# AlainSchoebi/semantic-bundle-adjustment-colmap

Measured on AMD Instinct MI355X. Metric: residuals+Jacobians/sec and BA-iteration wall-time, 1k cams / 1M pts / 10M obs, higher is better.
Workload: dtype f64

## Files before the change

semantic-bundle-adjustment-colmap_amd/csrc/semantic.hip:

```cpp
#include <hip/hip_runtime.h>

#include <map>

#include <algorithm>
#include <cmath>
#include <cstring>
#include <type_traits>

#include "ba_math.h"
#include "kernels.h"
#include "semantic.h"

namespace miba {

namespace {

constexpr double kMinStep = 1.4901161193847656e-08;

struct SemArgs {
  const SemSample* samples;
  const SemPair* pairs;
  const double* qt;
  const double* cam;
  const uint32_t* img_cam;
// ... 148 lines not shown
  Q[0] = aa + bb - cc - dd; Q[1] = 2.0 * (bc - ad);  Q[2] = 2.0 * (ac + bd);
  Q[3] = 2.0 * (bc + ad);  Q[4] = aa - bb + cc - dd; Q[5] = 2.0 * (cd - ab);
  Q[6] = 2.0 * (bd - ac);  Q[7] = 2.0 * (ab + cd);  Q[8] = aa - bb - cc + dd;
}

[[maybe_unused]] __device__ inline double rcp_refined(double x) {
  double r = __builtin_amdgcn_rcp(x);
  r = fma(r, fma(-x, r, 1.0), r);
  r = fma(r, fma(-x, r, 1.0), r);
  return r;
}

template <int M>
__device__ inline double distortion_gain(const double* K, double r2) {
  constexpr int np = Model<M>::kNumParams;
  double s = 0.0;
  if constexpr (M == kSimpleRadial || M == kRadial) {
#pragma unroll
    for (int k = 3; k < np; ++k) s += fabs(K[k]);
  } else if constexpr (M == kOpenCV) {
#pragma unroll
    for (int k = 4; k < np; ++k) s += fabs(K[k]);
  }
  const double g = 1.0 + r2;
  return 1.0 + s * g * g * g;
}

template <int M>
__device__ inline void world_to_image_fma(const double* K, double u, double v, double* x, double* y) {
#pragma clang fp contract(fast)
  if constexpr (M == kSimplePinhole) {
    *x = K[0] * u + K[1];
    *y = K[0] * v + K[2];
  } else if constexpr (M == kPinhole) {
    *x = K[0] * u + K[2];
    *y = K[1] * v + K[3];
  } else if constexpr (M == kSimpleRadial || M == kRadial) {
    const double r2 = u * u + v * v;
    double rad = K[3] * r2;
    if constexpr (M == kRadial) rad = rad + K[4] * r2 * r2;
    *x = K[0] * (u + u * rad) + K[1];
    *y = K[0] * (v + v * rad) + K[2];
  } else {
    const double k1 = K[4], k2 = K[5], p1 = K[6], p2 = K[7];
    const double u2 = u * u, uv = u * v, v2 = v * v, r2 = u2 + v2;
    const double rad = k1 * r2 + k2 * r2 * r2;
    const double du = u * rad + 2.0 * p1 * uv + p2 * (r2 + 2.0 * u2);
    const double dv = v * rad + 2.0 * p2 * uv + p1 * (r2 + 2.0 * v2);
    *x = K[0] * (u + du) + K[2];
    *y = K[1] * (v + dv) + K[3];
  }
}

__device__ inline void matvec3_t_fma(const double* A, double v0, double v1, double v2, const double* t,
                                     double pp[3]) {
#pragma clang fp contract(fast)
#pragma unroll
  for (int c = 0; c < 3; ++c) pp[c] = A[3 * c] * v0 + A[3 * c + 1] * v1 + A[3 * c + 2] * v2 + t[c];
}

template <int M>
__device__ inline double margin_model_term(const double* K2, const double p[3], double mag) {
  const double iz = 1.0 / p[2];
  const double u = p[0] * iz, v = p[1] * iz;
  return 2e-11 * (fabs(K2[0]) + fabs(K2[1])) * distortion_gain<M>(K2, u * u + v * v) * (1.0 + fabs(u) + fabs(v)) *
         (1.0 + mag * fabs(iz));
}

template <int M, bool FAST = false>
__device__ inline bool resolve(const SemArgs& a, const double p[3], double mag, float label1, const double* K2,
                               const float2* dl2, const PixelCache& pc, double& f, double exk = 0.0) {
  double iz;
  if constexpr (FAST) {
    const double x0 = p[2];
    double r = __builtin_amdgcn_rcp(x0);
    iz = fma(r, fma(-x0, r, 1.0), r);
  } else {
    iz = rcp_refined(p[2]);
  }
  const double u = p[0] * iz, v = p[1] * iz;
  double x, y;
  if constexpr (FAST)
    world_to_image_fma<M>(K2, u, v, &x, &y);
  else
    world_to_image<M>(K2, u, v, &x, &y);
  if (!(fabs(x) < 1e8 && fabs(y) < 1e8 && fabs(u) < 1e6 && fabs(v) < 1e6)) return false;
  double ex;
  if constexpr (FAST) {
    ex = 1e-6 + exk + 1e-11 * (fabs(x) + fabs(y));
  } else {
    const double kscale = (fabs(K2[0]) + fabs(K2[1])) * distortion_gain<M>(K2, u * u + v * v) *
                          (1.0 + fabs(u) + fabs(v)) * (1.0 + mag * fabs(iz));
    ex = 1e-6 + 1e-11 * (kscale + fabs(x) + fabs(y));
  }
  const double fx = floor(x), fy = floor(y);
  const double rx = x - fx, ry = y - fy;
  if (!(fabs(rx - 0.5) > ex && fabs(ry - 0.5) > ex)) return false;
  const int px = (int)fx + (rx > 0.5 ? 1 : 0);
  const int py = (int)fy + (ry > 0.5 ? 1 : 0);
  if (px < 0 || px >= a.W || py < 0 || py >= a.H) {
    f = 0.0;
    return true;
  }
  float2 s;
  if (pc.valid && px == pc.px && py == pc.py) {
    s = make_float2(pc.depth, pc.label);
  } else {
    s = dl2[(size_t)py * a.W + px];
  }
  const double dd = fabs((double)s.x - p[2]) - a.threshold;
  if (!(fabs(dd) > 1e-9 * (1.0 + fabs((double)s.x) + mag))) return false;
  f = (dd > 0.0) ? 0.0 : ((label1 == s.y) ? 0.0 : 1.0);
  return true;
}

struct PairConst {
  double q1[4], t1[3], q2[4], t2[3];
  double uqi[4];
  double ti[3];
  double u2[4];
  double R2[9];
  double C[9];
  double K2[8];
  uint32_t var1, var2, mask1, mask2;
  uint32_t slot, H2, W2, TW2;
  uint64_t roff, toff;
  double pert[28];
  double ood[14];
  double A[16][9];
  double pj[8][3];
  double rho1, rho2, dt1[3], dt2[3];
};

__device__ __forceinline__ SemArgs with_pair(const SemArgs& ak, const PairConst* __restrict__ P) {
  SemArgs a = ak;
  a.H = (int)P->H2;
  a.W = (int)P->W2;
  a.TW = (int)P->TW2;
  return a;
}

__device__ inline void stencil_bounds(const double* q, const double* t, double rel_step, double* rho, double dt[3]) {
  const double nq2 = q[0] * q[0] + q[1] * q[1] + q[2] * q[2] + q[3] * q[3];
  const double nq = sqrt(nq2);
  double r = 0.0;
  for (int k = 0; k < 4; ++k) {
    const double delta = fmax(kMinStep, fabs(q[k]) * rel_step);
    const double d = fmax(fabs((q[k] + delta) - q[k]), fabs(q[k] - (q[k] - delta)));
    const double perp = d * sqrt(fmax(0.0, 1.0 - q[k] * q[k] / nq2));
    const double den = nq - d;
    r = fmax(r, den > 0.0 ? 2.0 * perp / den : INFINITY);
  }
  *rho = r * 1.001;
  for (int k = 0; k < 3; ++k) {
    const double delta = fmax(kMinStep, fabs(t[k]) * rel_step);
    dt[k] = fmax(fabs((t[k] + delta) - t[k]), fabs(t[k] - (t[k] - delta))) * 1.001;
  }
}

__device__ inline void stencil_prep(const double* q1, const double* t1, const double* q2, const double* t2,
                                    double rel_step, int e, PairConst* __restrict__ P) {
  const int m = e >> 1;
  const bool minus = e & 1;
  const int grp = m < 4 ? 0 : (m < 7 ? 1 : (m < 11 ? 2 : 3));
  const int k = m - (grp == 0 ? 0 : (grp == 1 ? 4 : (grp == 2 ? 7 : 11)));
  const double orig = grp == 0 ? q1[k] : (grp == 1 ? t1[k] : (grp == 2 ? q2[k] : t2[k]));
  const double delta = fmax(kMinStep, fabs(orig) * rel_step);
  const double pert = minus ? orig - delta : orig + delta;
  P->pert[e] = pert;
  if (minus) {
    double one_over_delta = 1.0 / delta;
    one_over_delta /= 2;
    P->ood[m] = one_over_delta;
  }
  if (grp == 1 || grp == 3) return;
  const double* q = grp == 0 ? q1 : q2;
  double qq[4] = {q[0], q[1], q[2], q[3]};
  qq[k] = pert;
  double Q[9];
  quat_matrix_un(qq, Q);
  const double in = 1.0 / (qq[0] * qq[0] + qq[1] * qq[1] + qq[2] * qq[2] + qq[3] * qq[3]);
  double* A = P->A[grp == 0 ? e : e - 6];
  if (grp == 0) {
    double u2[4], R2[9];
// ... 24 lines not shown
  const int lane = threadIdx.x & 31;
  if (zero_n && blockIdx.x == 0 && (int)threadIdx.x < nzero) zero_n[threadIdx.x] = 0u;
  if (k >= npairs) return;
  for (int e = lane; e < blk_stride; e += 32) pair_blk[(size_t)k * blk_stride + e] = 0.0;
  if (pair_cnt && lane == 31) pair_cnt[k] = 0u;
  if (lane > 28) return;
  const SemPair pr = pairs[k];
  if (lane < 28) {
    const double* a1 = qt + 8 * (size_t)pr.i;
    const double* a2 = qt + 8 * (size_t)pr.j;
    const double q1[4] = {a1[0], a1[1], a1[2], a1[3]}, t1[3] = {a1[4], a1[5], a1[6]};
    const double q2[4] = {a2[0], a2[1], a2[2], a2[3]}, t2[3] = {a2[4], a2[5], a2[6]};
    stencil_prep(q1, t1, q2, t2, rel_step, lane, out + k);
    return;
  }
  PairConst& P = out[k];
  const double* a1 = qt + 8 * (size_t)pr.i;
  const double* a2 = qt + 8 * (size_t)pr.j;
  for (int m = 0; m < 4; ++m) { P.q1[m] = a1[m]; P.q2[m] = a2[m]; }
  for (int m = 0; m < 3; ++m) { P.t1[m] = a1[4 + m]; P.t2[m] = a2[4 + m]; }
  Pose1Stage s;
  const double zero[3] = {0.0, 0.0, 0.0};
  pose1_stage(P.q1, zero, s);
  {
    const double* q1 = P.q1;
    const double sc = 1.0 / sqrt(q1[0] * q1[0] + q1[1] * q1[1] + q1[2] * q1[2] + q1[3] * q1[3]);
    const double qi[4] = {sc * q1[0], -(sc * q1[1]), -(sc * q1[2]), -(sc * q1[3])};
    const double scale = 1.0 / sqrt(qi[0] * qi[0] + qi[1] * qi[1] + qi[2] * qi[2] + qi[3] * qi[3]);
    for (int m = 0; m < 4; ++m) P.uqi[m] = scale * qi[m];
  }
  P.ti[0] = -(s.R[0] * P.t1[0] + s.R[1] * P.t1[1] + s.R[2] * P.t1[2]);
  P.ti[1] = -(s.R[3] * P.t1[0] + s.R[4] * P.t1[1] + s.R[5] * P.t1[2]);
  P.ti[2] = -(s.R[6] * P.t1[0] + s.R[7] * P.t1[1] + s.R[8] * P.t1[2]);
  unit_quat(P.q2, P.u2);
  unit_quat_matrix(P.u2, P.R2);
  for (int r = 0; r < 3; ++r)
    for (int c = 0; c < 3; ++c)
      P.C[3 * r + c] = P.R2[3 * r] * s.R[c] + P.R2[3 * r + 1] * s.R[3 + c] + P.R2[3 * r + 2] * s.R[6 + c];
  const double* K = cam + 8 * (size_t)img_cam[pr.j];
  for (int m = 0; m < 8; ++m) P.K2[m] = K[m];
  P.var1 = pr.var1;
  P.var2 = pr.var2;
  P.mask1 = (img_flags[pr.i] >> 1) & 7u;
  P.mask2 = (img_flags[pr.j] >> 1) & 7u;
  P.slot = raster_slot[pr.j];
  const SlotInfo si = slots[P.slot];
  P.H2 = (uint32_t)si.H;
  P.W2 = (uint32_t)si.W;
  P.TW2 = (uint32_t)si.TW;
  P.roff = si.off;
  P.toff = si.toff;
  stencil_bounds(P.q1, P.t1, rel_step, &P.rho1, P.dt1);
  stencil_bounds(P.q2, P.t2, rel_step, &P.rho2, P.dt2);
}

constexpr int kPairVals = 78 + 12;
constexpr int kPairStride = 96;
constexpr int kSemRow = 13;

template <int M>
__device__ __forceinline__ double stencil_reference(const SemArgs& a, const PairConst* __restrict__ P, int grp, int k,
                                                 double pert, const double pc1[3], float label1, const double* K2,
                                                 const float2* dl2) {
  double qq1[4], tt1[3], qq2[4], tt2[3];
#pragma unroll
  for (int c = 0; c < 4; ++c) {
    qq1[c] = (grp == 0 && c == k) ? pert : P->q1[c];
    qq2[c] = (grp == 2 && c == k) ? pert : P->q2[c];
  }
#pragma unroll
  for (int c = 0; c < 3; ++c) {
    tt1[c] = (grp == 1 && c == k) ? pert : P->t1[c];
    tt2[c] = (grp == 3 && c == k) ? pert : P->t2[c];
  }
  int st2;
  return semantic_error<M>(a, pc1, label1, qq1, tt1, qq2, tt2, K2, dl2, &st2);
}

template <bool FAST, int GRP>
__device__ __forceinline__ void stencil_pp(const PairConst* __restrict__ P, int e, int k, const double w[3],
                                           const double pw[3], const double p2[3], double pp[3]) {
  if constexpr (GRP == 0 || GRP == 2) {
    const double* A = P->A[GRP == 0 ? e : e - 6];
    const double* v = GRP == 0 ? w : pw;
    if constexpr (FAST) {
      matvec3_t_fma(A, v[0], v[1], v[2], P->t2, pp);
    } else {
#pragma unroll
      for (int c = 0; c < 3; ++c) pp[c] = A[3 * c] * v[0] + A[3 * c + 1] * v[1] + A[3 * c + 2] * v[2] + P->t2[c];
    }
  } else if constexpr (GRP == 1) {
    const double dt = P->pert[e] - P->t1[k];
#pragma unroll
    for (int c = 0; c < 3; ++c) pp[c] = p2[c] - dt * P->C[3 * c + k];
  } else {
    const double dt = P->pert[e] - P->t2[k];
#pragma unroll
    for (int c = 0; c < 3; ++c) pp[c] = p2[c] + (c == k ? dt : 0.0);
  }
}

template <int M, bool FAST, int GRP>
__device__ __forceinline__ double stencil_point(const SemArgs& a, const PairConst* __restrict__ P, int e, int k,
                                                const double w[3], const double pw[3], const double p2[3],
                                                double mag, const double pc1[3], float label1, const double* K2,
                                                const float2* dl2, const PixelCache& pc, double exk) {
// ... 370 lines not shown
  for (int k = 0; k < nc; ++k) gm = fmax(gm, fmax(cu[k], cv[k]));
  if (!(gm < 0.1)) return false;
  const double ru = fabs(u) + gm, rv = fabs(v) + gm;
  const double H = second_derivative_bound<M>(K2, sqrt(ru * ru + rv * rv) * (1.0 + 1e-12));
  const double fx = fabs(K2[0]);
  const double fy = (M == kPinhole || M == kOpenCV) ? fabs(K2[1]) : fabs(K2[0]);
  double bxm = 0.0, bym = 0.0;
  for (int k = 0; k < nc; ++k) {
    const double sk = cu[k] + cv[k];
    bxm = fmax(bxm, (fabs(A[0]) + fx * H * sk) * cu[k] + (fabs(A[1]) + fx * H * sk) * cv[k]);
    bym = fmax(bym, (fabs(A[2]) + fy * H * sk) * cu[k] + (fabs(A[3]) + fy * H * sk) * cv[k]);
  }
  const double gain = distortion_gain<M>(K2, u * u + v * v);
  const double kscale = (fabs(K2[0]) + fabs(K2[1])) * gain * (1.0 + fabs(u) + fabs(v)) * (1.0 + c.mag * fabs(iz));
  const double ex = 1e-6 + 1e-11 * (kscale + fabs(x) + fabs(y));
  const double bx = bxm * (1.0 + 1e-12) + ex;
  const double by = bym * (1.0 + 1e-12) + ex;
  fb.x0 = (int)round(x - bx);
  fb.y0 = (int)round(y - by);
  fb.ncol = (int)round(x + bx) - fb.x0 + 1;
  fb.nrow = (int)round(y + by) - fb.y0 + 1;
  fb.d = az_max;
  return fb.ncol <= 3 && fb.nrow <= 3;
}

template <int M>
__device__ __forceinline__ void image_jac_bound(const double* K, double u, double v, double Ah[4]) {
  const double r2 = u * u + v * v, r1 = fabs(u) + fabs(v);
  if constexpr (M == kSimplePinhole) {
    Ah[0] = Ah[3] = fabs(K[0]);
    Ah[1] = Ah[2] = 0.0;
  } else if constexpr (M == kPinhole) {
    Ah[0] = fabs(K[0]);
    Ah[3] = fabs(K[1]);
    Ah[1] = Ah[2] = 0.0;
  } else if constexpr (M == kSimpleRadial) {
    const double k = fabs(K[3]);
    Ah[0] = Ah[3] = fabs(K[0]) * (1.0 + 3.0 * k * r2);
    Ah[1] = Ah[2] = fabs(K[0]) * (k * r2);
  } else if constexpr (M == kRadial) {
    const double k1 = fabs(K[3]), k2 = fabs(K[4]);
    Ah[0] = Ah[3] = fabs(K[0]) * (1.0 + 3.0 * k1 * r2 + 5.0 * k2 * r2 * r2);
    Ah[1] = Ah[2] = fabs(K[0]) * (k1 * r2 + 2.0 * k2 * r2 * r2);
  } else {
    const double k1 = fabs(K[4]), k2 = fabs(K[5]), p1 = fabs(K[6]), p2 = fabs(K[7]);
    const double rad = 3.0 * k1 * r2 + 5.0 * k2 * r2 * r2, off = k1 * r2 + 2.0 * k2 * r2 * r2 + 2.0 * (p1 + p2) * r1;
    Ah[0] = fabs(K[0]) * (1.0 + rad + (2.0 * p1 + 6.0 * p2) * r1);
    Ah[1] = fabs(K[0]) * off;
    Ah[2] = fabs(K[1]) * off;
    Ah[3] = fabs(K[1]) * (1.0 + rad + (6.0 * p1 + 2.0 * p2) * r1);
  }
}

template <int M, bool EXACT_A = false, bool GROUPS = false>
__device__ __forceinline__ bool flat_box_coarse(const PairConst* __restrict__ P, const Centre& c, const double* K2,
                                                double u, double v, double x, double y, FlatBox& fb) {
  const double z = c.p2[2];
  if (!(z > 0.0)) return false;
  double Ae[4];
  if constexpr (EXACT_A) {
    constexpr int np = Model<M>::kNumParams;
    double Jp[2 * np];
    world_to_image_jac<M>(K2, u, v, &x, &y, Ae, Jp);
  }
  if (!(fabs(x) < 1e8 && fabs(y) < 1e8 && fabs(u) < 1e6 && fabs(v) < 1e6)) return false;
  double dq = 0.0, tx = 0.0, ty = 0.0, tz = 0.0;
  if (P->var1) {
    dq = P->rho1 * sqrt(c.w[0] * c.w[0] + c.w[1] * c.w[1] + c.w[2] * c.w[2]) * (1.0 + 1e-12);
    tx = fmax(P->dt1[0] * fabs(P->C[0]), fmax(P->dt1[1] * fabs(P->C[1]), P->dt1[2] * fabs(P->C[2])));
    ty = fmax(P->dt1[0] * fabs(P->C[3]), fmax(P->dt1[1] * fabs(P->C[4]), P->dt1[2] * fabs(P->C[5])));
    tz = fmax(P->dt1[0] * fabs(P->C[6]), fmax(P->dt1[1] * fabs(P->C[7]), P->dt1[2] * fabs(P->C[8])));
  }
  if (P->var2) {
    dq = fmax(dq, P->rho2 * sqrt(c.pw[0] * c.pw[0] + c.pw[1] * c.pw[1] + c.pw[2] * c.pw[2]) * (1.0 + 1e-12));
    tx = fmax(tx, P->dt2[0]);
    ty = fmax(ty, P->dt2[1]);
    tz = fmax(tz, P->dt2[2]);
  }
  const double az = fmax(dq, tz);
  if (!(z - az > 0.5 * z)) return false;
  const double iden = 1.0 / (z - az) * (1.0 + 1e-12);
  const double cu_r = (dq + fabs(u) * dq) * iden, cv_r = (dq + fabs(v) * dq) * iden;
  const double cu_t = (tx + fabs(u) * tz) * iden, cv_t = (ty + fabs(v) * tz) * iden;
  const double cu = fmax(cu_r, cu_t), cv = fmax(cv_r, cv_t);
  const double gm = fmax(cu, cv);
  if (!(gm < 0.1)) return false;
  const double ru = fabs(u) + gm, rv = fabs(v) + gm;
  const double H = second_derivative_bound<M>(K2, sqrt(ru * ru + rv * rv) * (1.0 + 1e-12));
  const double fx = fabs(K2[0]);
  const double fy = (M == kPinhole || M == kOpenCV) ? fabs(K2[1]) : fabs(K2[0]);
  double Ah[4];
  if constexpr (EXACT_A) {
#pragma unroll
    for (int k = 0; k < 4; ++k) Ah[k] = fabs(Ae[k]);
  } else {
    image_jac_bound<M>(K2, u, v, Ah);
  }
  double bxm, bym;
  if constexpr (GROUPS) {
    const double sr = cu_r + cv_r, st = cu_t + cv_t;
    bxm = fmax((Ah[0] + fx * H * sr) * cu_r + (Ah[1] + fx * H * sr) * cv_r,
               (Ah[0] + fx * H * st) * cu_t + (Ah[1] + fx * H * st) * cv_t);
    bym = fmax((Ah[2] + fy * H * sr) * cu_r + (Ah[3] + fy * H * sr) * cv_r,
               (Ah[2] + fy * H * st) * cu_t + (Ah[3] + fy * H * st) * cv_t);
  } else {
    const double sk = cu + cv;
    bxm = (Ah[0] + fx * H * sk) * cu + (Ah[1] + fx * H * sk) * cv;
    bym = (Ah[2] + fy * H * sk) * cu + (Ah[3] + fy * H * sk) * cv;
  }
  const double gain = distortion_gain<M>(K2, u * u + v * v);
  const double kscale = (fabs(K2[0]) + fabs(K2[1])) * gain * (1.0 + fabs(u) + fabs(v)) * (1.0 + c.mag * fabs(1.0 / z));
  const double ex = 1e-6 + 1e-11 * (kscale + fabs(x) + fabs(y));
  const double bx = bxm * (1.0 + 1e-12) + ex;
  const double by = bym * (1.0 + 1e-12) + ex;
  fb.x0 = (int)round(x - bx);
  fb.y0 = (int)round(y - by);
  fb.ncol = (int)round(x + bx) - fb.x0 + 1;
  fb.nrow = (int)round(y + by) - fb.y0 + 1;
  fb.d = az;
  return fb.ncol <= 3 && fb.nrow <= 3;
}

__device__ __forceinline__ int flat_index(const SemArgs& a, const FlatBox& fb, bool cand, int q) {
  const int px = fb.x0 + q % 3, py = fb.y0 + q / 3;
  const bool in = cand && q % 3 < fb.ncol && q / 3 < fb.nrow && px >= 0 && px < a.W && py >= 0 && py < a.H;
  return in ? py * a.W + px : 0;
}

__device__ __forceinline__ bool flat_check(const SemArgs& a, const FlatBox& fb, const float2 s[9], double z,
                                           double mag, float label1, double r) {
  bool flat = true;
#pragma unroll
  for (int q = 0; q < 9; ++q) {
    const int px = fb.x0 + q % 3, py = fb.y0 + q / 3;
    if (q % 3 < fb.ncol && q / 3 < fb.nrow) {
      double f = 0.0;
      if (px >= 0 && px < a.W && py >= 0 && py < a.H) {
        const double dz = fabs((double)s[q].x - z) - a.threshold;
        if (!(fabs(dz) > fb.d + 1e-9 * (1.0 + fabs((double)s[q].x) + mag))) flat = false;
        f = dz > 0.0 ? 0.0 : (label1 == s[q].y ? 0.0 : 1.0);
      }
      if (f != r) flat = false;
    }
  }
  return flat;
}

template <int M>
__device__ __forceinline__ bool stencil_flat(const SemArgs& a, const PairConst* __restrict__ P, const Centre& c,
                                             float label1, const double* K2, const float2* __restrict__ dl2) {
  FlatBox fb;
  if (!flat_box<M>(P, c, K2, fb)) return false;
  float2 s[9];
#pragma unroll
  for (int q = 0; q < 9; ++q) s[q] = dl2[flat_index(a, fb, true, q)];
  return flat_check(a, fb, s, c.p2[2], c.mag, label1, c.r);
}

template <int M, bool FAST = false, int NB = 0, bool FLAT = false>
__global__ __launch_bounds__(kBlock) void semantic_linearize_kernel(SemArgs ak, const SemTile* __restrict__ tiles,
                                                                     const PairConst* __restrict__ pcs,
                                                                     double* __restrict__ pair_blk,
                                                                     double* __restrict__ cost_partial,
                                                                     double* __restrict__ r_out,
                                                                     int32_t* __restrict__ status_out,
                                                                     double* __restrict__ J_out, int write_samples) {
  constexpr int kHalf = kBlock / 2;
  constexpr int kBuf = FLAT ? kBlock * 12 : kHalf * kSemRow;
  __shared__ double sbuf[kBuf];
  __shared__ double spart[2 * kPairVals];
  __shared__ double sred[4];
// ... 181 lines not shown
    if (cur == 0ull) {
      const unsigned long long prev = atomicCAS(keys + h, 0ull, key);
      if (prev == 0ull || prev == key) return;
    }
  }
  atomicOr(overflow, 1u);
}

__global__ __launch_bounds__(256) void label_index_kernel(const float2* __restrict__ dl, int64_t n,
                                                          const unsigned long long* __restrict__ keys,
                                                          uint8_t* __restrict__ lab8) {
  const int64_t k = (int64_t)blockIdx.x * 256 + threadIdx.x;
  if (k >= n) return;
  const uint32_t bits = __float_as_uint(dl[k].y);
  const unsigned long long key = (unsigned long long)bits | (1ull << 32);
  uint32_t h = pal_hash(bits);
  for (int probe = 0; probe < 256 && keys[h] != key; ++probe) h = (h + 1u) & 255u;
  lab8[k] = (uint8_t)h;
}

__global__ __launch_bounds__(256) void depth_tile_kernel(const float2* __restrict__ dl,
                                                         const SlotInfo* __restrict__ slots, float2* __restrict__ out) {
  const SlotInfo si = slots[blockIdx.y];
  const int H = si.H, W = si.W, TW = si.TW, TH = (H + 7) / 8;
  const int rem = (int)(blockIdx.x * 256 + threadIdx.x);
  if (rem >= TH * TW) return;
  const int64_t k = (int64_t)si.toff + rem;
  const int ty = rem / TW, tx = rem - ty * TW;
  const float2* base = dl + si.off;
  float dmin = __builtin_inff(), dmax = -__builtin_inff();
  bool nan = false;
  const int y1 = min(8 * ty + 10, H), x1 = min(8 * tx + 10, W);
  for (int y = 8 * ty; y < y1; ++y)
    for (int x = 8 * tx; x < x1; ++x) {
      const float d = base[(int64_t)y * W + x].x;
      nan = nan || d != d;
      dmin = fminf(dmin, d);
      dmax = fmaxf(dmax, d);
    }
  out[k] = nan ? make_float2(__builtin_nanf(""), __builtin_nanf("")) : make_float2(dmin, dmax);
}

__device__ __forceinline__ int tile_depth_side(const SemArgs& a, const FlatBox& fb, float2 dr, double z, double mag) {
  const double dmin = (double)dr.x, dmax = (double)dr.y;
  if (!(dmin <= dmax)) return 0;
  const double margin = fb.d + 1e-9 * (1.0 + fmax(fabs(dmin), fabs(dmax)) + mag);
  const double far = fmax(fabs(dmax - z), fabs(dmin - z));
  if (a.threshold - far > margin) return 1;
  const double nearest = (z >= dmin && z <= dmax) ? 0.0 : fmin(fabs(dmin - z), fabs(dmax - z));
  if (nearest - a.threshold > margin) return 2;
  return 0;
}

template <int M, bool FAST, bool WS = false, bool LP = false, int COARSE = 0>
__global__ __launch_bounds__(kBlock) void semantic_flat_kernel(SemArgs ak, const SemTile* __restrict__ tiles,
                                                               const PairConst* __restrict__ pcs,
                                                               unsigned long long* __restrict__ dmask,
                                                               double* __restrict__ cost_partial,
                                                               double* __restrict__ r_out,
                                                               int32_t* __restrict__ status_out,
                                                               double* __restrict__ J_out, int write_samples) {
  __shared__ double sred[kBlock / 64];
  __shared__ float spal[LP ? 256 : 1];
  const SemTile t = tiles[blockIdx.x];
  const PairConst* __restrict__ P = pcs + t.pair;
  const SemArgs a = with_pair(ak, P);
  const int tid = threadIdx.x, lane = tid & 63;
  const bool active = tid < (int)t.count;
  const int64_t n = (int64_t)t.start + tid;
  const float2* dl2 = a.dl + P->roff;
  const double* K2 = P->K2;
  double cost = 0.0;
  bool deferred = false;
  if constexpr (LP) {
    static_assert(kBlock >= 256, "one palette entry per thread");
    spal[tid] = a.pal[tid];
    __syncthreads();
  }
  if (active) {
    const SemSample smp = a.samples[n];
    Centre c;
    double rot[3];
    unit_quat_rotate(P->uqi, smp.pc1, rot);
    c.pw[0] = rot[0] + P->ti[0];
    c.pw[1] = rot[1] + P->ti[1];
    c.pw[2] = rot[2] + P->ti[2];
    double rot2[3];
    unit_quat_rotate(P->u2, c.pw, rot2);
    c.p2[0] = rot2[0] + P->t2[0];
    c.p2[1] = rot2[1] + P->t2[1];
    c.p2[2] = rot2[2] + P->t2[2];
    c.mag = fabs(smp.pc1[0]) + fabs(smp.pc1[1]) + fabs(smp.pc1[2]) + fabs(P->t1[0]) + fabs(P->t1[1]) +
            fabs(P->t1[2]) + fabs(c.pw[0]) + fabs(c.pw[1]) + fabs(c.pw[2]) + fabs(P->t2[0]) + fabs(P->t2[1]) +
            fabs(P->t2[2]);
    c.w[0] = smp.pc1[0] - P->t1[0];
    c.w[1] = smp.pc1[1] - P->t1[1];
    c.w[2] = smp.pc1[2] - P->t1[2];
    const double u2 = c.p2[0] / c.p2[2];
    const double v2 = c.p2[1] / c.p2[2];
    double x2, y2;
    world_to_image<M>(K2, u2, v2, &x2, &y2);
    const int cpx = cast_to_int_x86(round(x2));
    const int cpy = cast_to_int_x86(round(y2));
    const bool cin = !(cpx < 0 || cpx >= a.W || cpy < 0 || cpy >= a.H);
    FlatBox fb;
    const bool cand = COARSE == 3   ? flat_box_coarse<M, false, true>(P, c, K2, u2, v2, x2, y2, fb)
                      : COARSE == 2 ? flat_box_coarse<M, true>(P, c, K2, u2, v2, x2, y2, fb)
                      : COARSE == 1 ? flat_box_coarse<M>(P, c, K2, u2, v2, x2, y2, fb)
                                    : flat_box<M>(P, c, K2, fb);
    bool decided = false;
    bool resolved = false;
    if constexpr (LP) {
      if (cand && fb.x0 >= 0 && fb.y0 >= 0 && fb.x0 + fb.ncol <= a.W && fb.y0 + fb.nrow <= a.H && cpx >= fb.x0 &&
          cpx < fb.x0 + fb.ncol && cpy >= fb.y0 && cpy < fb.y0 + fb.nrow) {
        const float2 dr = a.dtile[P->toff + (size_t)(fb.y0 >> 3) * a.TW + (fb.x0 >> 3)];
        const uint8_t* lp = a.lab8 + P->roff + (size_t)fb.y0 * a.W + fb.x0;
        const uint8_t lc = lp[(size_t)(cpy - fb.y0) * a.W + (cpx - fb.x0)];
        uint8_t L[9];
#pragma unroll
        for (int q = 0; q < 9; ++q) L[q] = (q % 3 < fb.ncol && q / 3 < fb.nrow) ? lp[(size_t)(q / 3) * a.W + q % 3] : lc;
        const int side = tile_depth_side(a, fb, dr, c.p2[2], c.mag);
        if (side == 2) {
          c.st = MI_BA_INVALID_DEPTH;
          c.r = 0.0;
          decided = resolved = true;
        } else if (side == 1) {
          c.st = MI_BA_VALID;
          c.r = (smp.label1 == spal[lc]) ? 0.0 : 1.0;
          bool flat = true;
#pragma unroll
          for (int q = 0; q < 9; ++q) flat = flat && ((smp.label1 == spal[L[q]]) ? 0.0 : 1.0) == c.r;
          resolved = true;
          decided = flat;
          deferred = !flat;
        }
      }
    }
    if constexpr (WS) {
      if (!resolved && cand && fb.x0 >= 0 && fb.y0 >= 0 && fb.x0 + 2 < a.W && fb.y0 + 2 < a.H) {
        const float4 w = a.wsum[P->roff + (size_t)fb.y0 * a.W + fb.x0];
        decided = resolved = window_decides(a, fb, w, c.p2[2], c.mag, smp.label1, &c.st, &c.r);
      }
    }
    if (!resolved && cand &&
        (fb.x0 + fb.ncol <= 0 || fb.x0 >= a.W || fb.y0 + fb.nrow <= 0 || fb.y0 >= a.H)) {
      c.st = MI_BA_OUT_OF_BOUNDS;
      c.r = 0.0;
      decided = resolved = true;
    }
    if (!resolved) {
      const float2 sc = dl2[cin ? cpy * a.W + cpx : 0];
      float2 s[9];
#pragma unroll
      for (int q = 0; q < 9; ++q) s[q] = dl2[flat_index(a, fb, cand, q)];
      if (!cin) {
        c.st = MI_BA_OUT_OF_BOUNDS;
        c.r = 0.0;
      } else if (fabs((double)sc.x - c.p2[2]) > a.threshold) {
        c.st = MI_BA_INVALID_DEPTH;
        c.r = 0.0;
      } else {
        c.st = MI_BA_VALID;
        c.r = (smp.label1 == sc.y) ? 0.0 : 1.0;
      }
      deferred = !(cand && flat_check(a, fb, s, c.p2[2], c.mag, smp.label1, c.r));
    }
    double rho[3];
    loss_eval(a.loss_type, a.loss_scale, c.r * c.r, rho);
    cost = 0.5 * (a.weight * rho[0]);
    if (write_samples) {
      r_out[n] = c.r;
      status_out[n] = c.st + ((write_samples & 2) && deferred ? 0x1000 : 0) + ((write_samples & 4) && decided ? 0x4000 : 0);
      if (!deferred) {
        double2* jo = reinterpret_cast<double2*>(J_out + 12 * n);
#pragma unroll
        for (int m = 0; m < 6; ++m) jo[m] = make_double2(0.0, 0.0);
      }
    }
  }
  const unsigned long long bal = __ballot(deferred);
  if (lane == 0) dmask[(size_t)blockIdx.x * (kBlock / 64) + (tid >> 6)] = bal;
  double v = cost;
  for (int off = 32; off > 0; off >>= 1) v += __shfl_xor(v, off, 64);
  if (lane == 0) sred[tid >> 6] = v;
  __syncthreads();
  if (tid == 0) {
    double s = 0.0;
#pragma unroll
    for (int w = 0; w < kBlock / 64; ++w) s += sred[w];
    cost_partial[blockIdx.x] = s;
  }
}

template <int M, bool FAST, int NB, bool BOX = false, int WPE = 1>
__global__ __launch_bounds__(64, WPE) void semantic_deferred_kernel(SemArgs ak, const uint2* __restrict__ chunks,
                                                              const uint32_t* __restrict__ ccount,
                                                              const PairConst* __restrict__ pcs,
                                                              const uint32_t* __restrict__ pair_cnt,
                                                              const uint32_t* __restrict__ dlist,
                                                              const uint32_t* __restrict__ pair_chunk0,
                                                              double* __restrict__ cpart,
                                                              double* __restrict__ J_out, int write_samples,
                                                              int32_t* __restrict__ status_out = nullptr) {
  __shared__ double sJ[64 * kSemRow];
  __shared__ float2 sbox[BOX ? 64 * 9 : 1];
  const uint32_t nch = ccount ? *ccount : blockIdx.x + 1;
  const uint32_t stride = ccount ? gridDim.x : 1u;
  for (uint32_t ci = blockIdx.x; ci < nch; ci += stride) {
  const uint2 ch = chunks[ci];
  const uint32_t cnt = pair_cnt[ch.x];
  if (ch.y >= cnt) continue;
  const PairConst* __restrict__ P = pcs + ch.x;
  const SemArgs a = with_pair(ak, P);
  const int lane = threadIdx.x;
  const uint32_t k = ch.y + lane;
  const uint32_t pstart = a.pairs[ch.x].start;
  const float2* dl2 = a.dl + P->roff;
  const double* K2 = P->K2;
  double rowv[kSemRow];
#pragma unroll
  for (int q = 0; q < kSemRow; ++q) rowv[q] = 0.0;
  if (k < cnt) {
    const int64_t n = (int64_t)pstart + dlist[pstart + k];
    const SemSample smp = a.samples[n];
    Centre c;
// ... 1015 lines not shown
```

Measured before the change: 18.93 billion.

## Streamline flat-pixel classifier with precomputed pair bounds and fast approximate math

The per-sample centre projection now uses the precomputed composite rotation C as a single matvec, plus hardware reciprocal with one Newton step and a float sqrt upper bound, instead of two quaternion rotations and exact division. Per-pair stencil bounds and camera-magnitude terms are hoisted into PairConst. The bound routine is merged into one templated function with widened safety margins. Samples near rounding or threshold boundaries fall back to the exact reference path, which trades fewer FLOPs per sample for extra branches and more code.

```diff
diff --git a/semantic-bundle-adjustment-colmap_amd/csrc/semantic.hip b/semantic-bundle-adjustment-colmap_amd/csrc/semantic.hip
--- a/semantic-bundle-adjustment-colmap_amd/csrc/semantic.hip
+++ b/semantic-bundle-adjustment-colmap_amd/csrc/semantic.hip
@@ -224,6 +224,61 @@
   }
 }
 
+template <int M>
+__device__ __forceinline__ void image_point_jac_fma(const double* K, double u, double v, double* x, double* y,
+                                                    double A[4], double* r2o) {
+#pragma clang fp contract(fast)
+  const double u2 = u * u, v2 = v * v, r2 = u2 + v2;
+  *r2o = r2;
+  if constexpr (M == kSimplePinhole) {
+    *x = K[0] * u + K[1];
+    *y = K[0] * v + K[2];
+    A[0] = A[3] = K[0];
+    A[1] = A[2] = 0.0;
+  } else if constexpr (M == kPinhole) {
+    *x = K[0] * u + K[2];
+    *y = K[1] * v + K[3];
+    A[0] = K[0];
+    A[3] = K[1];
+    A[1] = A[2] = 0.0;
+  } else if constexpr (M == kSimpleRadial || M == kRadial) {
+    const double f = K[0];
+    double rad = K[3] * r2, g = 2.0 * K[3];
+    if constexpr (M == kRadial) {
+      rad = rad + K[4] * r2 * r2;
+      g = g + 4.0 * K[4] * r2;
+    }
+    *x = f * (u + u * rad) + K[1];
+    *y = f * (v + v * rad) + K[2];
+    const double guv = g * u * v;
+    A[0] = f * (1.0 + rad + g * u2);
+    A[1] = A[2] = f * guv;
+    A[3] = f * (1.0 + rad + g * v2);
+  } else {
+    const double k1 = K[4], k2 = K[5], p1 = K[6], p2 = K[7];
+    const double uv = u * v;
+    const double rad = r2 * (k1 + k2 * r2);
+    const double g = 2.0 * k1 + 4.0 * k2 * r2;
+    const double tp = 2.0 * (p1 * u + p2 * v);
+    *x = K[0] * (u + u * rad + 2.0 * p1 * uv + p2 * (r2 + 2.0 * u2)) + K[2];
+    *y = K[1] * (v + v * rad + 2.0 * p2 * uv + p1 * (r2 + 2.0 * v2)) + K[3];
+    const double off = g * uv + tp;
+    A[0] = K[0] * (1.0 + rad + g * u2 + 2.0 * p1 * v + 6.0 * p2 * u);
+    A[1] = K[0] * off;
+    A[2] = K[1] * off;
+    A[3] = K[1] * (1.0 + rad + g * v2 + 2.0 * p2 * u + 6.0 * p1 * v);
+  }
+}
+
+__device__ __forceinline__ double rcp_newton1(double x) {
+  const double r = __builtin_amdgcn_rcp(x);
+  return fma(r, fma(-x, r, 1.0), r);
+}
+
+__device__ __forceinline__ double sqrt_upper(double s) {
+  return fma((double)__builtin_amdgcn_sqrtf((float)s), 1.0 + 1e-6, 1e-18);
+}
+
 __device__ inline void matvec3_t_fma(const double* A, double v0, double v1, double v2, const double* t,
                                      double pp[3]) {
 #pragma clang fp contract(fast)
@@ -302,6 +357,11 @@
   double A[16][9];
   double pj[8][3];
   double rho1, rho2, dt1[3], dt2[3];
+  double frho, ftx, fty, ftz;
+  double fk01;
+  double fks[3];
+  double fh6[2], fh20[2], fh3;
+  double ft12;
 };
 
 __device__ __forceinline__ SemArgs with_pair(const SemArgs& ak, const PairConst* __restrict__ P) {
@@ -432,6 +492,33 @@
   P.toff = si.toff;
   stencil_bounds(P.q1, P.t1, rel_step, &P.rho1, P.dt1);
   stencil_bounds(P.q2, P.t2, rel_step, &P.rho2, P.dt2);
+  double rho = 0.0, tx = 0.0, ty = 0.0, tz = 0.0;
+  if (pr.var1) {
+    rho = P.rho1;
+    tx = fmax(P.dt1[0] * fabs(P.C[0]), fmax(P.dt1[1] * fabs(P.C[1]), P.dt1[2] * fabs(P.C[2])));
+    ty = fmax(P.dt1[0] * fabs(P.C[3]), fmax(P.dt1[1] * fabs(P.C[4]), P.dt1[2] * fabs(P.C[5])));
+    tz = fmax(P.dt1[0] * fabs(P.C[6]), fmax(P.dt1[1] * fabs(P.C[7]), P.dt1[2] * fabs(P.C[8])));
+  }
+  if (pr.var2) {
+    rho = fmax(rho, P.rho2);
+    tx = fmax(tx, P.dt2[0]);
+    ty = fmax(ty, P.dt2[1]);
+    tz = fmax(tz, P.dt2[2]);
+  }
+  P.frho = rho;
+  P.ftx = tx;
+  P.fty = ty;
+  P.ftz = tz;
+  P.fk01 = fabs(K[0]) + fabs(K[1]);
+  P.fks[0] = fabs(K[3]);
+  P.fks[1] = fabs(K[3]) + fabs(K[4]);
+  P.fks[2] = fabs(K[4]) + fabs(K[5]) + fabs(K[6]) + fabs(K[7]);
+  P.fh6[0] = 6.0 * fabs(K[3]);
+  P.fh6[1] = 6.0 * fabs(K[4]);
+  P.fh20[0] = 20.0 * fabs(K[4]);
+  P.fh20[1] = 20.0 * fabs(K[5]);
+  P.fh3 = 6.0 * (fabs(K[6]) + fabs(K[7]));
+  P.ft12 = fabs(P.t1[0]) + fabs(P.t1[1]) + fabs(P.t1[2]) + fabs(P.t2[0]) + fabs(P.t2[1]) + fabs(P.t2[2]);
 }
 
 constexpr int kPairVals = 78 + 12;
@@ -908,71 +995,101 @@
   }
 }
 
-template <int M, bool EXACT_A = false, bool GROUPS = false>
-__device__ __forceinline__ bool flat_box_coarse(const PairConst* __restrict__ P, const Centre& c, const double* K2,
-                                                double u, double v, double x, double y, FlatBox& fb) {
-  const double z = c.p2[2];
+struct FlatCentre {
+  double z, u, v, x, y, A[4];
+  double nw;
+  double mag;
+  double m1;
+  double ex;
+};
+
+template <int M, int COARSE>
+__device__ __forceinline__ bool flat_bound(const PairConst* __restrict__ P, const double* K2, const FlatCentre& c,
+                                           FlatBox& fb) {
+#pragma clang fp contract(fast)
+  const double z = c.z;
   if (!(z > 0.0)) return false;
-  double Ae[4];
-  if constexpr (EXACT_A) {
-    constexpr int np = Model<M>::kNumParams;
-    double Jp[2 * np];
-    world_to_image_jac<M>(K2, u, v, &x, &y, Ae, Jp);
-  }
-  if (!(fabs(x) < 1e8 && fabs(y) < 1e8 && fabs(u) < 1e6 && fabs(v) < 1e6)) return false;
-  double dq = 0.0, tx = 0.0, ty = 0.0, tz = 0.0;
-  if (P->var1) {
-    dq = P->rho1 * sqrt(c.w[0] * c.w[0] + c.w[1] * c.w[1] + c.w[2] * c.w[2]) * (1.0 + 1e-12);
-    tx = fmax(P->dt1[0] * fabs(P->C[0]), fmax(P->dt1[1] * fabs(P->C[1]), P->dt1[2] * fabs(P->C[2])));
-    ty = fmax(P->dt1[0] * fabs(P->C[3]), fmax(P->dt1[1] * fabs(P->C[4]), P->dt1[2] * fabs(P->C[5])));
-    tz = fmax(P->dt1[0] * fabs(P->C[6]), fmax(P->dt1[1] * fabs(P->C[7]), P->dt1[2] * fabs(P->C[8])));
-  }
-  if (P->var2) {
-    dq = fmax(dq, P->rho2 * sqrt(c.pw[0] * c.pw[0] + c.pw[1] * c.pw[1] + c.pw[2] * c.pw[2]) * (1.0 + 1e-12));
-    tx = fmax(tx, P->dt2[0]);
-    ty = fmax(ty, P->dt2[1]);
-    tz = fmax(tz, P->dt2[2]);
-  }
-  const double az = fmax(dq, tz);
-  if (!(z - az > 0.5 * z)) return false;
-  const double iden = 1.0 / (z - az) * (1.0 + 1e-12);
-  const double cu_r = (dq + fabs(u) * dq) * iden, cv_r = (dq + fabs(v) * dq) * iden;
-  const double cu_t = (tx + fabs(u) * tz) * iden, cv_t = (ty + fabs(v) * tz) * iden;
-  const double cu = fmax(cu_r, cu_t), cv = fmax(cv_r, cv_t);
-  const double gm = fmax(cu, cv);
-  if (!(gm < 0.1)) return false;
-  const double ru = fabs(u) + gm, rv = fabs(v) + gm;
-  const double H = second_derivative_bound<M>(K2, sqrt(ru * ru + rv * rv) * (1.0 + 1e-12));
+  if (!(fabs(c.x) < 1e8 && fabs(c.y) < 1e8 && fabs(c.u) < 1e6 && fabs(c.v) < 1e6 && c.m1 < 1e3)) return false;
+  const double dq = P->frho * c.nw;
+  const double az = fmax(dq, P->ftz);
+  const double zl = (z - az) - 1e-11 * c.mag;
+  if (!(zl > 0.5 * z)) return false;
+  const double iden = rcp_newton1(zl) * (1.0 + 1e-9);
+  const double eu = 1e-8 * fabs(c.u) + 1e-8, ev = 1e-8 * fabs(c.v) + 1e-8;
+  const double ua = fabs(c.u) + eu, va = fabs(c.v) + ev;
   const double fx = fabs(K2[0]);
   const double fy = (M == kPinhole || M == kOpenCV) ? fabs(K2[1]) : fabs(K2[0]);
+  auto second = [&](double gm) {
+    const double ru = ua + gm, rv = va + gm;
+    const double rho = sqrt_upper(ru * ru + rv * rv);
+    if constexpr (M == kSimpleRadial) return P->fh6[0] * rho;
+    else if constexpr (M == kRadial) return P->fh6[0] * rho + P->fh20[0] * rho * rho * rho;
+    else if constexpr (M == kOpenCV) return P->fh6[1] * rho + P->fh20[1] * rho * rho * rho + P->fh3;
+    else return 0.0;
+  };
   double Ah[4];
-  if constexpr (EXACT_A) {
-#pragma unroll
-    for (int k = 0; k < 4; ++k) Ah[k] = fabs(Ae[k]);
+  if constexpr (COARSE == 1 || COARSE == 3) {
+    image_jac_bound<M>(K2, ua, va, Ah);
   } else {
-    image_jac_bound<M>(K2, u, v, Ah);
+#pragma unroll
+    for (int k = 0; k < 4; ++k) Ah[k] = fabs(c.A[k]);
   }
   double bxm, bym;
-  if constexpr (GROUPS) {
-    const double sr = cu_r + cv_r, st = cu_t + cv_t;
-    bxm = fmax((Ah[0] + fx * H * sr) * cu_r + (Ah[1] + fx * H * sr) * cv_r,
-               (Ah[0] + fx * H * st) * cu_t + (Ah[1] + fx * H * st) * cv_t);
-    bym = fmax((Ah[2] + fy * H * sr) * cu_r + (Ah[3] + fy * H * sr) * cv_r,
-               (Ah[2] + fy * H * st) * cu_t + (Ah[3] + fy * H * st) * cv_t);
+  if constexpr (COARSE == 0) {
+    double cu[7], cv[7];
+    int nc = 0;
+    auto cls = [&](double ax, double ay, double azk) {
+      cu[nc] = (ax + ua * azk) * iden + eu;
+      cv[nc] = (ay + va * azk) * iden + ev;
+      ++nc;
+    };
+    cls(dq, dq, dq);
+    if (P->var1) {
+#pragma unroll
+      for (int k = 0; k < 3; ++k)
+        cls(P->dt1[k] * fabs(P->C[k]), P->dt1[k] * fabs(P->C[3 + k]), P->dt1[k] * fabs(P->C[6 + k]));
+    }
+    if (P->var2) {
+      cls(P->dt2[0], 0.0, 0.0);
+      cls(0.0, P->dt2[1], 0.0);
+      cls(0.0, 0.0, P->dt2[2]);
+    }
+    double gm = 0.0;
+    for (int k = 0; k < nc; ++k) gm = fmax(gm, fmax(cu[k], cv[k]));
+    if (!(gm < 0.1)) return false;
+    const double H = second(gm);
+    bxm = bym = 0.0;
+    for (int k = 0; k < nc; ++k) {
+      const double sk = cu[k] + cv[k];
+      bxm = fmax(bxm, (Ah[0] + fx * H * sk) * cu[k] + (Ah[1] + fx * H * sk) * cv[k]);
+      bym = fmax(bym, (Ah[2] + fy * H * sk) * cu[k] + (Ah[3] + fy * H * sk) * cv[k]);
+    }
   } else {
-    const double sk = cu + cv;
-    bxm = (Ah[0] + fx * H * sk) * cu + (Ah[1] + fx * H * sk) * cv;
-    bym = (Ah[2] + fy * H * sk) * cu + (Ah[3] + fy * H * sk) * cv;
-  }
-  const double gain = distortion_gain<M>(K2, u * u + v * v);
-  const double kscale = (fabs(K2[0]) + fabs(K2[1])) * gain * (1.0 + fabs(u) + fabs(v)) * (1.0 + c.mag * fabs(1.0 / z));
-  const double ex = 1e-6 + 1e-11 * (kscale + fabs(x) + fabs(y));
-  const double bx = bxm * (1.0 + 1e-12) + ex;
-  const double by = bym * (1.0 + 1e-12) + ex;
-  fb.x0 = (int)round(x - bx);
-  fb.y0 = (int)round(y - by);
-  fb.ncol = (int)round(x + bx) - fb.x0 + 1;
-  fb.nrow = (int)round(y + by) - fb.y0 + 1;
+    const double cu_r = (dq + ua * dq) * iden + eu, cv_r = (dq + va * dq) * iden + ev;
+    const double cu_t = (P->ftx + ua * P->ftz) * iden + eu, cv_t = (P->fty + va * P->ftz) * iden + ev;
+    const double cu = fmax(cu_r, cu_t), cv = fmax(cv_r, cv_t);
+    const double gm = fmax(cu, cv);
+    if (!(gm < 0.1)) return false;
+    const double H = second(gm);
+    const double hx = fx * H, hy = fy * H;
+    if constexpr (COARSE == 3) {
+      const double sr = cu_r + cv_r, st = cu_t + cv_t;
+      bxm = fmax((Ah[0] + hx * sr) * cu_r + (Ah[1] + hx * sr) * cv_r,
+                 (Ah[0] + hx * st) * cu_t + (Ah[1] + hx * st) * cv_t);
+      bym = fmax((Ah[2] + hy * sr) * cu_r + (Ah[3] + hy * sr) * cv_r,
+                 (Ah[2] + hy * st) * cu_t + (Ah[3] + hy * st) * cv_t);
+    } else {
+      const double sk = cu + cv;
+      bxm = (Ah[0] + hx * sk) * cu + (Ah[1] + hx * sk) * cv;
+      bym = (Ah[2] + hy * sk) * cu + (Ah[3] + hy * sk) * cv;
+    }
+  }
+  const double bx = bxm * (1.0 + 1e-9) + 2.0 * c.ex;
+  const double by = bym * (1.0 + 1e-9) + 2.0 * c.ex;
+  fb.x0 = (int)floor((c.x - bx) + 0.5);
+  fb.y0 = (int)floor((c.y - by) + 0.5);
+  fb.ncol = (int)floor((c.x + bx) + 0.5) - fb.x0 + 1;
+  fb.nrow = (int)floor((c.y + by) + 0.5) - fb.y0 + 1;
   fb.d = az;
   return fb.ncol <= 3 && fb.nrow <= 3;
 }
@@ -1260,6 +1377,18 @@
   return 0;
 }
 
+__device__ __forceinline__ void reference_point(const PairConst* __restrict__ P, const double pc1[3], double p2[3]) {
+  double rot[3], pw[3], rot2[3];
+  unit_quat_rotate(P->uqi, pc1, rot);
+  pw[0] = rot[0] + P->ti[0];
+  pw[1] = rot[1] + P->ti[1];
+  pw[2] = rot[2] + P->ti[2];
+  unit_quat_rotate(P->u2, pw, rot2);
+  p2[0] = rot2[0] + P->t2[0];
+  p2[1] = rot2[1] + P->t2[1];
+  p2[2] = rot2[2] + P->t2[2];
+}
+
 template <int M, bool FAST, bool WS = false, bool LP = false, int COARSE = 0>
 __global__ __launch_bounds__(kBlock) void semantic_flat_kernel(SemArgs ak, const SemTile* __restrict__ tiles,
                                                                const PairConst* __restrict__ pcs,
@@ -1287,35 +1416,56 @@
   }
   if (active) {
     const SemSample smp = a.samples[n];
-    Centre c;
-    double rot[3];
-    unit_quat_rotate(P->uqi, smp.pc1, rot);
-    c.pw[0] = rot[0] + P->ti[0];
-    c.pw[1] = rot[1] + P->ti[1];
-    c.pw[2] = rot[2] + P->ti[2];
-    double rot2[3];
-    unit_quat_rotate(P->u2, c.pw, rot2);
-    c.p2[0] = rot2[0] + P->t2[0];
-    c.p2[1] = rot2[1] + P->t2[1];
-    c.p2[2] = rot2[2] + P->t2[2];
-    c.mag = fabs(smp.pc1[0]) + fabs(smp.pc1[1]) + fabs(smp.pc1[2]) + fabs(P->t1[0]) + fabs(P->t1[1]) +
-            fabs(P->t1[2]) + fabs(c.pw[0]) + fabs(c.pw[1]) + fabs(c.pw[2]) + fabs(P->t2[0]) + fabs(P->t2[1]) +
-            fabs(P->t2[2]);
-    c.w[0] = smp.pc1[0] - P->t1[0];
-    c.w[1] = smp.pc1[1] - P->t1[1];
-    c.w[2] = smp.pc1[2] - P->t1[2];
-    const double u2 = c.p2[0] / c.p2[2];
-    const double v2 = c.p2[1] / c.p2[2];
-    double x2, y2;
-    world_to_image<M>(K2, u2, v2, &x2, &y2);
-    const int cpx = cast_to_int_x86(round(x2));
-    const int cpy = cast_to_int_x86(round(y2));
+    const double w0 = smp.pc1[0] - P->t1[0], w1 = smp.pc1[1] - P->t1[1], w2 = smp.pc1[2] - P->t1[2];
+    FlatCentre fc;
+    fc.nw = sqrt_upper(fma(w2, w2, fma(w1, w1, w0 * w0)));
+    fc.mag = fma(1.7321, fc.nw, fabs(smp.pc1[0]) + fabs(smp.pc1[1]) + fabs(smp.pc1[2]) + P->ft12);
+    int st = 0;
+    double r = 0.0;
+    double p2[3];
+    matvec3_t_fma(P->C, w0, w1, w2, P->t2, p2);
+    double iz = rcp_newton1(p2[2]);
+    fc.u = p2[0] * iz;
+    fc.v = p2[1] * iz;
+    double r2;
+    image_point_jac_fma<M>(K2, fc.u, fc.v, &fc.x, &fc.y, fc.A, &r2);
+    int cpx, cpy;
+    bool slow;
+    {
+      fc.m1 = fma(fc.mag, fabs(iz), 1.0);
+      const double g1 = 1.0 + r2;
+      const double ks = (M == kSimpleRadial ? P->fks[0] : M == kRadial ? P->fks[1] : M == kOpenCV ? P->fks[2] : 0.0);
+      const double gain = fma(ks, g1 * g1 * g1, 1.0);
+      const double kscale = P->fk01 * gain * (1.0 + fabs(fc.u) + fabs(fc.v)) * fc.m1;
+      fc.ex = 1e-6 + fma(2e-11, kscale, 1e-11 * (fabs(fc.x) + fabs(fc.y)));
+      const double fx = floor(fc.x), fy = floor(fc.y);
+      const double rx = fc.x - fx, ry = fc.y - fy;
+      slow = !(fabs(fc.x) < 1e8 && fabs(fc.y) < 1e8 && fabs(fc.u) < 1e6 && fabs(fc.v) < 1e6 &&
+               fabs(rx - 0.5) > fc.ex && fabs(ry - 0.5) > fc.ex);
+      cpx = (int)fx + (rx > 0.5 ? 1 : 0);
+      cpy = (int)fy + (ry > 0.5 ? 1 : 0);
+    }
+    if (slow) {
+      reference_point(P, smp.pc1, p2);
+      fc.u = p2[0] / p2[2];
+      fc.v = p2[1] / p2[2];
+      double xf, yf;
+      image_point_jac_fma<M>(K2, fc.u, fc.v, &xf, &yf, fc.A, &r2);
+      world_to_image<M>(K2, fc.u, fc.v, &fc.x, &fc.y);
+      cpx = cast_to_int_x86(round(fc.x));
+      cpy = cast_to_int_x86(round(fc.y));
+      if (!(fc.ex < 1e300)) {
+        fc.m1 = fma(fc.mag, fabs(1.0 / p2[2]), 1.0);
+        fc.ex = 1e-6 + 2e-11 * P->fk01 * distortion_gain<M>(K2, fc.u * fc.u + fc.v * fc.v) *
+                           (1.0 + fabs(fc.u) + fabs(fc.v)) * fc.m1 + 1e-11 * (fabs(fc.x) + fabs(fc.y));
+      }
+    }
+    fc.z = p2[2];
+    bool exact_z = false;
+    float cdepth = 0.f, clabel = 0.f;
     const bool cin = !(cpx < 0 || cpx >= a.W || cpy < 0 || cpy >= a.H);
     FlatBox fb;
-    const bool cand = COARSE == 3   ? flat_box_coarse<M, false, true>(P, c, K2, u2, v2, x2, y2, fb)
-                      : COARSE == 2 ? flat_box_coarse<M, true>(P, c, K2, u2, v2, x2, y2, fb)
-                      : COARSE == 1 ? flat_box_coarse<M>(P, c, K2, u2, v2, x2, y2, fb)
-                                    : flat_box<M>(P, c, K2, fb);
+    const bool cand = flat_bound<M, COARSE>(P, K2, fc, fb);
     bool decided = false;
     bool resolved = false;
     if constexpr (LP) {
@@ -1327,17 +1477,17 @@
         uint8_t L[9];
 #pragma unroll
         for (int q = 0; q < 9; ++q) L[q] = (q % 3 < fb.ncol && q / 3 < fb.nrow) ? lp[(size_t)(q / 3) * a.W + q % 3] : lc;
-        const int side = tile_depth_side(a, fb, dr, c.p2[2], c.mag);
+        const int side = tile_depth_side(a, fb, dr, fc.z, fc.mag);
         if (side == 2) {
-          c.st = MI_BA_INVALID_DEPTH;
-          c.r = 0.0;
+          st = MI_BA_INVALID_DEPTH;
+          r = 0.0;
           decided = resolved = true;
         } else if (side == 1) {
-          c.st = MI_BA_VALID;
-          c.r = (smp.label1 == spal[lc]) ? 0.0 : 1.0;
+          st = MI_BA_VALID;
+          r = (smp.label1 == spal[lc]) ? 0.0 : 1.0;
           bool flat = true;
 #pragma unroll
-          for (int q = 0; q < 9; ++q) flat = flat && ((smp.label1 == spal[L[q]]) ? 0.0 : 1.0) == c.r;
+          for (int q = 0; q < 9; ++q) flat = flat && ((smp.label1 == spal[L[q]]) ? 0.0 : 1.0) == r;
           resolved = true;
           decided = flat;
           deferred = !flat;
@@ -1347,13 +1497,13 @@
     if constexpr (WS) {
       if (!resolved && cand && fb.x0 >= 0 && fb.y0 >= 0 && fb.x0 + 2 < a.W && fb.y0 + 2 < a.H) {
         const float4 w = a.wsum[P->roff + (size_t)fb.y0 * a.W + fb.x0];
-        decided = resolved = window_decides(a, fb, w, c.p2[2], c.mag, smp.label1, &c.st, &c.r);
+        decided = resolved = window_decides(a, fb, w, fc.z, fc.mag, smp.label1, &st, &r);
       }
     }
     if (!resolved && cand &&
         (fb.x0 + fb.ncol <= 0 || fb.x0 >= a.W || fb.y0 + fb.nrow <= 0 || fb.y0 >= a.H)) {
-      c.st = MI_BA_OUT_OF_BOUNDS;
-      c.r = 0.0;
+      st = MI_BA_OUT_OF_BOUNDS;
+      r = 0.0;
       decided = resolved = true;
     }
     if (!resolved) {
@@ -1362,23 +1512,40 @@
 #pragma unroll
       for (int q = 0; q < 9; ++q) s[q] = dl2[flat_index(a, fb, cand, q)];
       if (!cin) {
-        c.st = MI_BA_OUT_OF_BOUNDS;
-        c.r = 0.0;
-      } else if (fabs((double)sc.x - c.p2[2]) > a.threshold) {
-        c.st = MI_BA_INVALID_DEPTH;
-        c.r = 0.0;
+        st = MI_BA_OUT_OF_BOUNDS;
+        r = 0.0;
       } else {
-        c.st = MI_BA_VALID;
-        c.r = (smp.label1 == sc.y) ? 0.0 : 1.0;
+        const double dd = fabs((double)sc.x - fc.z) - a.threshold;
+        exact_z = !slow && !(fabs(dd) > 1e-9 * (1.0 + fabs((double)sc.x) + fc.mag));
+        cdepth = sc.x;
+        clabel = sc.y;
+        if (slow ? fabs((double)sc.x - fc.z) > a.threshold : dd > 0.0) {
+          st = MI_BA_INVALID_DEPTH;
+          r = 0.0;
+        } else {
+          st = MI_BA_VALID;
+          r = (smp.label1 == sc.y) ? 0.0 : 1.0;
+        }
       }
-      deferred = !(cand && flat_check(a, fb, s, c.p2[2], c.mag, smp.label1, c.r));
+      deferred = exact_z || !(cand && flat_check(a, fb, s, fc.z, fc.mag, smp.label1, r));
+    }
+    if (exact_z) {
+      const SemSample again = a.samples[n];
+      reference_point(P, again.pc1, p2);
+      if (fabs((double)cdepth - p2[2]) > a.threshold) {
+        st = MI_BA_INVALID_DEPTH;
+        r = 0.0;
+      } else {
+        st = MI_BA_VALID;
+        r = (again.label1 == clabel) ? 0.0 : 1.0;
+      }
     }
     double rho[3];
-    loss_eval(a.loss_type, a.loss_scale, c.r * c.r, rho);
+    loss_eval(a.loss_type, a.loss_scale, r * r, rho);
     cost = 0.5 * (a.weight * rho[0]);
     if (write_samples) {
-      r_out[n] = c.r;
-      status_out[n] = c.st + ((write_samples & 2) && deferred ? 0x1000 : 0) + ((write_samples & 4) && decided ? 0x4000 : 0);
+      r_out[n] = r;
+      status_out[n] = st + ((write_samples & 2) && deferred ? 0x1000 : 0) + ((write_samples & 4) && decided ? 0x4000 : 0);
       if (!deferred) {
         double2* jo = reinterpret_cast<double2*>(J_out + 12 * n);
 #pragma unroll
```

After: 18.98 billion, median of 4. About the same (+0.3%).
